# yahoo/CaffeOnSpark

Hardware: AMD Instinct MI355X
Metric: images/sec (higher is better)
Workload: dtype bf16; 1 GPU; model=alexnet(bvlc_reference/CaffeNet), global_batch=256, parallelism=dp1

## Files before the change

### caffeonspark_amd/ops/csrc/elementwise.hip

```cpp

#include "common.h"

namespace cosamd {

typedef unsigned short u16;
typedef unsigned short u16x8 __attribute__((ext_vector_type(8)));
typedef unsigned short u16x4 __attribute__((ext_vector_type(4)));
typedef float f32x4 __attribute__((ext_vector_type(4)));

__device__ __forceinline__ float ldbf(const u16* p) {
  return bf2f(*reinterpret_cast<const bf16*>(p));
}
__device__ __forceinline__ void stbf(u16* p, float v) {
  bf16 b = f2bf(v);
  *p = *reinterpret_cast<u16*>(&b);
}


__global__ void relu_fwd_kernel(const u16* __restrict__ x, u16* __restrict__ y,
                                float slope, int64_t n8, int64_t n) {
  if (blockIdx.x == 0 && threadIdx.x == 0)
    for (int64_t k = n8 * 8; k < n; ++k) {
      float f = ldbf(x + k);
      stbf(y + k, f > 0.f ? f : f * slope);
// ... 121 lines not shown
       i < n; i += (int64_t)gridDim.x * blockDim.x)
    stbf(y + i, ldbf(a + i) * ldbf(b + i));
}


__global__ void sgd_update_kernel(float* __restrict__ p, const float* __restrict__ g,
                                  float* __restrict__ v, float lr, float mu,
                                  float wd, int64_t n4, int64_t n) {
  for (int64_t i = (int64_t)blockIdx.x * blockDim.x + threadIdx.x;
       i < n4; i += (int64_t)gridDim.x * blockDim.x) {
    if (i * 4 + 4 <= n) {
      f32x4 pv = *reinterpret_cast<f32x4*>(p + i * 4);
      f32x4 gv = *reinterpret_cast<const f32x4*>(g + i * 4);
      f32x4 vv = *reinterpret_cast<f32x4*>(v + i * 4);
#pragma unroll
      for (int j = 0; j < 4; ++j) {
        float gg = gv[j] + wd * pv[j];
        vv[j] = mu * vv[j] + lr * gg;
        pv[j] -= vv[j];
      }
      *reinterpret_cast<f32x4*>(v + i * 4) = vv;
      *reinterpret_cast<f32x4*>(p + i * 4) = pv;
    } else {
      for (int64_t k = i * 4; k < n; ++k) {
        float gg = g[k] + wd * p[k];
        v[k] = mu * v[k] + lr * gg;
        p[k] -= v[k];
      }
    }
  }
}


__global__ void bias_act_cast_kernel(const float* __restrict__ in,
                                     const float* __restrict__ bias,
                                     u16* __restrict__ out, int64_t rows,
                                     int cols, int relu) {
  int64_t total = rows * cols;
  for (int64_t i = (int64_t)blockIdx.x * blockDim.x + threadIdx.x;
       i < total; i += (int64_t)gridDim.x * blockDim.x) {
    float v = in[i];
    if (bias != nullptr) v += bias[i % cols];
    if (relu && v < 0.f) v = 0.f;
    stbf(out + i, v);
  }
}

void bias_act_cast(const float* in, const float* bias, void* out,
                   int64_t rows, int cols, bool relu, hipStream_t stream) {
  int64_t total = rows * cols;
  int blocks = (int)hmin<int64_t>(4096, (total + 255) / 256);
  bias_act_cast_kernel<<<blocks, 256, 0, stream>>>(
      in, bias, (u16*)out, rows, cols, relu ? 1 : 0);
}


__global__ void transpose_bf16_kernel(const u16* __restrict__ in,
                                      u16* __restrict__ out,
                                      int R, int C, int tiles_c) {
  __shared__ unsigned lds32[64][67];
  int nblk = gridDim.x;
  int tile = xcd_swizzle(blockIdx.x, nblk);
  int r0 = (tile / tiles_c) * 128;
  int c0 = (tile % tiles_c) * 64;
  int t = threadIdx.x;
  bool interior = (r0 + 128 <= R) && (c0 + 64 <= C);
  int lc8 = (t & 7) * 8;
#pragma unroll
  for (int half = 0; half < 2; ++half) {
    int r2 = (t >> 3) + half * 32;
    int grlo = r0 + 2 * r2, grhi = grlo + 1;
    if (interior) {
      u16x8 vlo = *reinterpret_cast<const u16x8*>(
          in + (int64_t)grlo * C + c0 + lc8);
      u16x8 vhi = *reinterpret_cast<const u16x8*>(
          in + (int64_t)grhi * C + c0 + lc8);
#pragma unroll
      for (int j = 0; j < 8; ++j)
        lds32[r2][lc8 + j] = (unsigned)vlo[j] | ((unsigned)vhi[j] << 16);
    } else {
#pragma unroll
      for (int j = 0; j < 8; ++j) {
        int gc = c0 + lc8 + j;
        u16 lo = (grlo < R && gc < C) ? in[(int64_t)grlo * C + gc] : 0;
        u16 hi = (grhi < R && gc < C) ? in[(int64_t)grhi * C + gc] : 0;
        lds32[r2][lc8 + j] = (unsigned)lo | ((unsigned)hi << 16);
      }
    }
  }
  __syncthreads();
  int cl = t >> 4;
  int lr8 = (t & 15) * 8;
#pragma unroll
  for (int pass = 0; pass < 4; ++pass) {
    int c = cl + pass * 16;
    int gc = c0 + c;
    if (interior) {
      u16x8 v;
#pragma unroll
      for (int m = 0; m < 4; ++m) {
        unsigned pair = lds32[(lr8 >> 1) + m][c];
        v[2 * m] = (u16)(pair & 0xFFFF);
        v[2 * m + 1] = (u16)(pair >> 16);
      }
      *reinterpret_cast<u16x8*>(out + (int64_t)gc * R + r0 + lr8) = v;
    } else if (gc < C) {
// ... 643 lines not shown
```

### caffeonspark_amd/ops/csrc/ext.cpp

```cpp

#include <torch/extension.h>
#include <ATen/hip/HIPContext.h>

#include <cstdint>

typedef struct ihipStream_t* hipStream_t;

namespace cosamd {

void gemm_bf16(const void* A, const void* B, void* C, const float* bias,
               int M, int N, int K, int lda, int ldb, int ldc,
               bool trans_a, bool trans_b, int store_mode, int splitk,
               bool relu, float alpha, int m_alloc, int n_alloc,
               hipStream_t stream);
void gemm_f32(const float* A, const float* B, float* C, const float* bias,
              int M, int N, int K, int64_t lda, int64_t ldb, int64_t ldc,
              bool trans_a, bool trans_b, int splitk, bool relu,
              hipStream_t stream);
void im2col_f32(const float* x, float* col, int N, int H, int W, int P,
                int Q, int R, int S, int sh, int sw, int ph, int pw, int dh,
                int dw, int c0, int Cg, int64_t sN, int64_t sC, int64_t sH,
                int64_t sW, hipStream_t stream);
void col2im_f32(const float* dcol, float* dx, int N, int H, int W, int P,
                int Q, int R, int S, int sh, int sw, int ph, int pw, int dh,
                int dw, int c0, int Cg, int64_t sN, int64_t sC, int64_t sH,
                int64_t sW, hipStream_t stream);
void gemm_conv_fwd(const void* X, const void* B, void* C,
                   const float* bias, const void* zpage, int M, int N,
                   int K, int ldb, int ldc, bool relu, bool accum,
                   const int* geom, int groups, int gs_c, int gs_b,
                   int gs_n, int cfg, int vec, hipStream_t stream);
struct ConvCfg { int id, bm, bn, waves, depth; };
ConvCfg conv_fwd_plan(int M, int N, int K);
int conv_fwd_num_cfgs();
ConvCfg conv_fwd_cfg(int id);
void gemm_conv_dw(const void* A, const void* X, float* C,
                  const void* zpage, int M, int N, int K, int lda, int ldc,
                  int store_mode, int splitk, float alpha, float* db,
                  const int* geom, hipStream_t stream);
void gemm_conv_fwd_sc(const void* X, const void* B, void* C,
                      const float* bias, int M, int N, int K, int ldb,
                      int ldc, bool relu, const int* geom,
                      hipStream_t stream);
void gemm_conv_dw_sc(const void* A, const void* X, float* C, int M,
                     int N, int K, int lda, int ldc, int store_mode,
                     int splitk, float alpha, float* db, const int* geom,
                     hipStream_t stream);
void repack_weights(const int64_t* table, int ndesc, int64_t max_total,
                    hipStream_t stream);
void dw_unpack_acc(const float* dwp, float* arena, int Kout, int Cg,
                   int R, int S, int Kpad, bool accumulate,
                   hipStream_t stream);
void s2d_pack(const void* x, void* out, int N, int H, int W, int C, int st,
              int ph, int pw, int Hp, int Wp, int64_t sN, int64_t sC,
              int64_t sH, int64_t sW, hipStream_t stream);
void s2d_pack_weight(const void* src, void* dst, int Kout, int Cg, int R,
                     int S, int st, int Kpad, hipStream_t stream);
void d2s_pack_weight(const void* src, void* dst, int Ci, int Co, int R,
                     int S, int st, int Kpad, hipStream_t stream);
void d2s_unpack(const void* z, void* y, int N, int Co, int Ho, int Wo,
                int st, int ph, int pw, int Hp, int Wp, int64_t sN,
                int64_t sC, int64_t sH, int64_t sW, hipStream_t stream);
void data_transform(const void* src, int64_t src_bytes, const int64_t* table,
                    const int64_t* table_host, int N, const float* mean,
                    int mean_mode, int64_t mean_numel, int mC, int mH,
                    int mW, float scale, void* out, bool out_bf16, int C,
                    int oh, int ow, int64_t osN, int64_t osC, int64_t osH,
// ... 107 lines not shown
                  int T, int N, int H, int n_alloc_whc, hipStream_t stream);
void lstm_seq_bwd(const void* dy, const void* w_hcT, const void* cont,
                  const void* h, const float* c, const float* act,
                  void* dxg, void* dh_rec, float* dh_f, float* dc_a,
                  float* dc_b, int T, int N, int H, int n_alloc_whcT,
                  hipStream_t stream);
int64_t lstm_step_lds_bytes(int N, int D, int H, int Ds);
void lstm_step(const void* x, const void* h_prev, const void* xs,
               const void* w_xc, const void* w_hc, const void* w_xsc,
               const void* bias, const float* cont, const float* c_prev,
               float* c_out, void* h_out, int N, int D, int H, int Ds,
               hipStream_t stream);
void softmax_loss_fwd(const void* x, const float* label, float* prob,
                      float* rowloss, float* loss, int* count,
                      int64_t nrows, int C, int ignore, bool has_ignore,
                      hipStream_t stream);
void softmax_loss_bwd(const float* prob, const float* label, void* dx,
                      float scale, int64_t nrows, int C, int ignore,
                      bool has_ignore, hipStream_t stream);

}

namespace {

using at::Tensor;

hipStream_t cur_stream() {
  return at::hip::getCurrentHIPStream().stream();
}

#define CHECK_BF16(t) \
  TORCH_CHECK((t).scalar_type() == at::kBFloat16, #t " must be bf16")
#define CHECK_F32(t) \
  TORCH_CHECK((t).scalar_type() == at::kFloat, #t " must be fp32")
#define CHECK_CUDA(t) TORCH_CHECK((t).is_cuda(), #t " must be on GPU")

void py_gemm(Tensor A, Tensor B, Tensor C, c10::optional<Tensor> bias,
             int64_t M, int64_t N, int64_t K, int64_t lda, int64_t ldb,
             int64_t ldc, bool trans_a, bool trans_b, int64_t store_mode,
             int64_t splitk, bool relu, double alpha, int64_t m_alloc,
             int64_t n_alloc) {
  CHECK_CUDA(A); CHECK_BF16(A); CHECK_BF16(B);
  const float* bptr = nullptr;
  if (bias.has_value()) {
    CHECK_F32(bias.value());
    bptr = bias.value().data_ptr<float>();
  }
  cosamd::gemm_bf16(
      A.data_ptr(), B.data_ptr(), C.data_ptr(), bptr, (int)M, (int)N, (int)K, (int)lda, (int)ldb, (int)ldc,
      trans_a, trans_b, (int)store_mode, (int)splitk, relu, (float)alpha,
      (int)m_alloc, (int)n_alloc, cur_stream());
}

int64_t span_f32(const Tensor& t) {
  return (int64_t)(t.storage().nbytes() / sizeof(float)) - t.storage_offset();
}

void py_gemm_f32(Tensor A, Tensor B, Tensor C, c10::optional<Tensor> bias,
                 int64_t M, int64_t N, int64_t K, int64_t lda, int64_t ldb,
                 int64_t ldc, bool trans_a, bool trans_b, int64_t splitk,
                 bool relu) {
  CHECK_CUDA(A); CHECK_CUDA(B); CHECK_CUDA(C);
  CHECK_F32(A); CHECK_F32(B); CHECK_F32(C);
  const int64_t lim = 1ll << 31;
  TORCH_CHECK(M > 0 && N > 0 && K > 0 && M < lim && N < lim && K < lim,
              "gemm_f32: bad M/N/K");
  int64_t ar = trans_a ? K : M, ac = trans_a ? M : K;
  int64_t br = trans_b ? K : N, bc = trans_b ? N : K;
  TORCH_CHECK(lda >= ac && ldb >= bc && ldc >= N,
              "gemm_f32: leading dimension smaller than the row");
  TORCH_CHECK((ar - 1) * lda + ac <= span_f32(A), "gemm_f32: A too small");
  TORCH_CHECK((br - 1) * ldb + bc <= span_f32(B), "gemm_f32: B too small");
  TORCH_CHECK((M - 1) * ldc + N <= span_f32(C), "gemm_f32: C too small");
  TORCH_CHECK(splitk >= 1 && splitk <= 65535, "gemm_f32: bad splitk");
  TORCH_CHECK((N + 127) / 128 <= 65535, "gemm_f32: N too large");
  const float* bptr = nullptr;
  if (bias.has_value()) {
    const Tensor& b = bias.value();
    CHECK_CUDA(b); CHECK_F32(b);
    TORCH_CHECK(b.is_contiguous() && b.numel() >= N,
                "gemm_f32: bias must hold N contiguous floats");
    bptr = b.data_ptr<float>();
  }
  cosamd::gemm_f32(A.data_ptr<float>(), B.data_ptr<float>(),
                   C.data_ptr<float>(), bptr, (int)M, (int)N, (int)K, lda,
                   ldb, ldc, trans_a, trans_b, (int)splitk, relu,
                   cur_stream());
}

void check_conv_f32(const Tensor& x, const Tensor& col, int64_t P, int64_t Q,
                    int64_t R, int64_t S, int64_t sh, int64_t sw, int64_t ph,
                    int64_t pw, int64_t dh, int64_t dw, int64_t c0,
                    int64_t Cg) {
  CHECK_CUDA(x); CHECK_CUDA(col); CHECK_F32(x); CHECK_F32(col);
  TORCH_CHECK(x.dim() == 4, "x must be 4-D");
  const int64_t lim = 1ll << 31;
  int64_t N = x.size(0), C = x.size(1), H = x.size(2), W = x.size(3);
  TORCH_CHECK(N > 0 && H > 0 && W > 0 && N < lim && H < lim && W < lim,
              "bad input shape");
  TORCH_CHECK(P > 0 && Q > 0 && R > 0 && S > 0 && sh > 0 && sw > 0 &&
              ph >= 0 && pw >= 0 && dh > 0 && dw > 0 && c0 >= 0 && Cg > 0 &&
              c0 + Cg <= C, "bad conv geometry");
  TORCH_CHECK(N * P * Q < lim && Cg * R * S < lim, "conv too large");
  int64_t last = 0;
  for (int d = 0; d < 4; ++d) {
    TORCH_CHECK(x.stride(d) >= 0, "negative stride");
// ... 603 lines not shown
                    dw.data_ptr<float>(), idx.numel(), dw.size(1), V,
                    cur_stream());
}

void py_lstm_seq_fwd(Tensor xg, Tensor w_hc, Tensor cont, Tensor h,
                     Tensor c, Tensor act, Tensor h_in, Tensor hg,
                     int64_t T, int64_t N, int64_t H, int64_t n_alloc) {
  CHECK_BF16(xg); CHECK_BF16(w_hc); CHECK_F32(c); CHECK_F32(act);
  CHECK_F32(hg);
  cosamd::lstm_seq_fwd(xg.data_ptr(), w_hc.data_ptr(), cont.data_ptr(),
                       h.data_ptr(), c.data_ptr<float>(),
                       act.data_ptr<float>(), h_in.data_ptr(),
                       hg.data_ptr<float>(), T, N, H, n_alloc,
                       cur_stream());
}

void py_lstm_seq_bwd(Tensor dy, Tensor w_hcT, Tensor cont, Tensor h,
                     Tensor c, Tensor act, Tensor dxg, Tensor dh_rec,
                     Tensor dh_f, Tensor dc_a, Tensor dc_b, int64_t T,
                     int64_t N, int64_t H, int64_t n_alloc) {
  CHECK_BF16(dy); CHECK_BF16(w_hcT); CHECK_F32(dh_f);
  cosamd::lstm_seq_bwd(dy.data_ptr(), w_hcT.data_ptr(), cont.data_ptr(),
                       h.data_ptr(), c.data_ptr<float>(),
                       act.data_ptr<float>(), dxg.data_ptr(),
                       dh_rec.data_ptr(), dh_f.data_ptr<float>(),
                       dc_a.data_ptr<float>(), dc_b.data_ptr<float>(),
                       T, N, H, n_alloc, cur_stream());
}

void py_softmax_loss_fwd(Tensor x, Tensor label, Tensor prob,
                         Tensor rowloss, Tensor loss, Tensor count,
                         int64_t ignore, bool has_ignore) {
  CHECK_BF16(x); CHECK_F32(label); CHECK_F32(prob); CHECK_F32(rowloss);
  TORCH_CHECK(rowloss.is_contiguous() && rowloss.numel() >= x.size(0),
              "rowloss must hold one value per row");
  cosamd::softmax_loss_fwd(x.data_ptr(), label.data_ptr<float>(),
                           prob.data_ptr<float>(),
                           rowloss.data_ptr<float>(), loss.data_ptr<float>(),
                           count.data_ptr<int>(), x.size(0), x.size(1),
                           (int)ignore, has_ignore, cur_stream());
}

void py_softmax_loss_bwd(Tensor prob, Tensor label, Tensor dx, double scale,
                         int64_t ignore, bool has_ignore) {
  cosamd::softmax_loss_bwd(prob.data_ptr<float>(), label.data_ptr<float>(),
                           dx.data_ptr(), scale, prob.size(0), prob.size(1),
                           (int)ignore, has_ignore, cur_stream());
}

}

PYBIND11_MODULE(TORCH_EXTENSION_NAME, m) {
  m.def("gemm", &py_gemm);
  m.def("gemm_f32", &py_gemm_f32);
  m.def("im2col_f32", &py_im2col_f32);
  m.def("col2im_f32", &py_col2im_f32);
  m.def("relu_colsum_bwd", &py_relu_colsum_bwd);
  m.def("relu_db_dense", &py_relu_db_dense);
  m.def("gemm_conv_fwd", &py_gemm_conv_fwd, py::arg("X"), py::arg("B"),
        py::arg("C"), py::arg("bias"), py::arg("zpage"), py::arg("M"),
        py::arg("N"), py::arg("K"), py::arg("ldb"), py::arg("ldc"),
        py::arg("relu"), py::arg("accum"), py::arg("geom"),
        py::arg("groups") = 1, py::arg("gs_c") = 0, py::arg("gs_b") = 0,
        py::arg("gs_n") = 0, py::arg("cfg") = -1, py::arg("vec") = -1);
  m.def("conv_fwd_plan", &py_conv_fwd_plan);
  m.def("conv_fwd_cfgs", &py_conv_fwd_cfgs);
  m.def("gemm_conv_dw", &py_gemm_conv_dw);
  m.def("gemm_conv_fwd_sc", &py_gemm_conv_fwd_sc);
  m.def("gemm_conv_dw_sc", &py_gemm_conv_dw_sc);
  m.def("im2col", &py_im2col);
  m.def("bn_stats", [](Tensor x, Tensor sum, Tensor sq, int64_t rows,
                       int64_t C) {
    cosamd::bn_stats(x.data_ptr(), sum.data_ptr<float>(),
                     sq.data_ptr<float>(), rows, C, cur_stream());
  });
  m.def("bn_bwd_sums", [](Tensor dy, Tensor xhat, Tensor s1, Tensor s2,
                          int64_t rows, int64_t C) {
    cosamd::bn_bwd_sums(dy.data_ptr(), xhat.data_ptr(),
                        s1.data_ptr<float>(), s2.data_ptr<float>(), rows,
                        C, cur_stream());
  });
  m.def("bn_norm", [](Tensor x, Tensor y, Tensor mean, Tensor invstd,
                      int64_t rows, int64_t C) {
    cosamd::bn_norm(x.data_ptr(), y.data_ptr(), mean.data_ptr<float>(),
                    invstd.data_ptr<float>(), rows, C, cur_stream());
  });
  m.def("bn_bwd", [](Tensor xhat, Tensor dy, Tensor dx, Tensor invstd,
                     Tensor s1, Tensor s2, double inv_m, int64_t rows,
                     int64_t C) {
    cosamd::bn_bwd(xhat.data_ptr(), dy.data_ptr(), dx.data_ptr(),
                   invstd.data_ptr<float>(), s1.data_ptr<float>(),
                   s2.data_ptr<float>(), (float)inv_m, rows, C,
                   cur_stream());
  });
  m.def("wino_conv", [](Tensor x, Tensor w, c10::optional<Tensor> bias,
                        Tensor y, Tensor U, Tensor V, Tensor M, int64_t N,
                        int64_t H, int64_t W, int64_t Cin, int64_t K,
                        int64_t wK, int64_t wC, int64_t u_rows_alloc,
                        bool flip, bool relu) {
    cosamd::wino_conv(x.data_ptr(), w.data_ptr<float>(),
                      bias ? bias->data_ptr<float>() : nullptr,
                      y.data_ptr(), U.data_ptr(), V.data_ptr(),
                      M.data_ptr(), N, H, W, Cin, K, wK, wC, u_rows_alloc,
                      flip, relu, cur_stream());
  });
  m.def("im2col_t", [](Tensor x, Tensor colT, int64_t N, int64_t H,
// ... 58 lines not shown
```

### caffeonspark_amd/ops/csrc/gemm.hip

```cpp

#include "common.h"

#include <type_traits>

namespace cosamd {

typedef __bf16 bf16x8 __attribute__((ext_vector_type(8)));
typedef unsigned short short8v __attribute__((ext_vector_type(8)));
typedef float f32x4 __attribute__((ext_vector_type(4)));

constexpr int BM = 128, BN = 128, BK = 32;
constexpr int NTHREADS = 256;

__device__ __forceinline__ int swz_chunk(int row, int chunk) {
  return chunk ^ ((row >> 1) & 3);
}


struct Tile { int bm, bn, tile_m, tile_n; };

template <int TBN, int TBM = BM>
__device__ __forceinline__ Tile decode_tile(int M, int N) {
  int mblocks = (M + TBM - 1) / TBM;
  int nblocks = (N + TBN - 1) / TBN;
// ... 123 lines not shown
        if (relu) {
#pragma unroll
          for (int j = 0; j < 8; ++j) v[j] = v[j] < 0.f ? 0.f : v[j];
        }
        short8v* dst =
            reinterpret_cast<short8v*>(C + (int64_t)grow * ldc + col);
        bf16 o[8];
        if (accum) {
          short8v old = *dst;
          __builtin_memcpy(o, &old, 16);
#pragma unroll
          for (int j = 0; j < 8; ++j) v[j] += bf2f(o[j]);
        }
#pragma unroll
        for (int j = 0; j < 8; ++j) o[j] = f2bf(v[j]);
        short8v out;
        __builtin_memcpy(&out, o, 16);
        *dst = out;
      }
    }
    __builtin_amdgcn_wave_barrier();
  }
}

template <int STORE, bool BIAS, int MF, int MROWS>
__device__ __forceinline__ void epilogue_f32(
    const f32x4 (&acc)[MF][4], float* C, const float* bias, int M, int N,
    int ldc, int tile_m, int tile_n, int wm, int wn, int lane, int relu,
    float alpha) {
  int crow0 = tile_m + wm * MROWS + ((lane >> 4) << 2);
  int ccol0 = tile_n + wn * 64 + (lane & 15);
#pragma unroll
  for (int fm = 0; fm < MF; ++fm) {
#pragma unroll
    for (int fn = 0; fn < 4; ++fn) {
      int col = ccol0 + fn * 16;
      if (col >= N) continue;
      float badd = (BIAS && bias != nullptr) ? bias[col] : 0.f;
#pragma unroll
      for (int r = 0; r < 4; ++r) {
        int row = crow0 + fm * 16 + r;
        if (row >= M) continue;
        float v = acc[fm][fn][r] * alpha;
        if (BIAS) {
          v += badd;
          if (relu && v < 0.f) v = 0.f;
        }
        if (STORE == 1)
          C[(int64_t)row * ldc + col] = v;
        else
          atomicAdd(C + (int64_t)row * ldc + col, v);
      }
    }
  }
}


__device__ __forceinline__ void stage_direct_guarded(
    bf16* lds_, const bf16* g_, int row0, int rows, int ld,
    int k0, int kend, int tid, int nthreads = NTHREADS) {
  auto* lds = reinterpret_cast<unsigned short*>(lds_);
  auto* g = reinterpret_cast<const unsigned short*>(g_);
  for (int slot = tid; slot < 512; slot += nthreads) {
    int row = slot >> 2;
    int kk = (slot & 3) * 8;
    int grow = row0 + row;
    int gk = k0 + kk;
    unsigned short* dst = lds + row * BK + (swz_chunk(row, slot & 3) << 3);
    if (grow < rows && gk + 8 <= kend && ((ld | gk) % 8 == 0)) {
      *reinterpret_cast<short8v*>(dst) =
          *reinterpret_cast<const short8v*>(g + (int64_t)grow * ld + gk);
    } else if (grow < rows) {
#pragma unroll
      for (int j = 0; j < 8; ++j)
        dst[j] = (gk + j < kend) ? g[(int64_t)grow * ld + gk + j] : 0;
    } else {
#pragma unroll
      for (int j = 0; j < 8; ++j) dst[j] = 0;
    }
  }
}


__device__ __forceinline__ void write_kpairs(
    unsigned short* lds, int m0, int kp, const unsigned short (&va)[8],
    const unsigned short (&vb)[8]) {
  int kk = kp * 2;
  int chunk0 = kk >> 3, kin = kk & 7;
#pragma unroll
  for (int j = 0; j < 8; ++j) {
    int row = m0 + j;
    unsigned int packed = (unsigned int)va[j] |
                          ((unsigned int)vb[j] << 16);
    *reinterpret_cast<unsigned int*>(
        lds + row * BK + (swz_chunk(row, chunk0) << 3) + kin) = packed;
  }
}

__device__ __forceinline__ void stage_trans_pair_guarded(
    bf16* lds_, const bf16* g_, int row0, int rows, int ld,
    int k0, int kend, int tid, int nthreads = NTHREADS,
    int tile_rows = BM) {
  auto* lds = reinterpret_cast<unsigned short*>(lds_);
  auto* g = reinterpret_cast<const unsigned short*>(g_);
  int rslots = tile_rows >> 3;
  int nslots = 16 * rslots;
// ... 971 lines not shown
  else
    gemm_conv_fwd_sc_kernel<4><<<grid, dim3(256), 0, stream>>>(
        (const bf16*)X, (const bf16*)B, (bf16*)C, bias, M, N, K, ldb,
        ldc, relu ? 1 : 0, gm);
}

void gemm_conv_dw_sc(const void* A, const void* X, float* C, int M,
                     int N, int K, int lda, int ldc, int store_mode,
                     int splitk, float alpha, float* db, const int* geom,
                     hipStream_t stream) {
  launch_wide_tt((const bf16*)A, C, M, N, K, lda, ldc, store_mode,
                 split_k(K, splitk), alpha, db,
                 BImplicitSC{(const bf16*)X, make_geom(geom)}, stream);
}

void gemm_conv_dw(const void* A, const void* X, float* C,
                  const void* zpage, int M, int N, int K, int lda, int ldc,
                  int store_mode, int splitk, float alpha, float* db,
                  const int* geom, hipStream_t stream) {
  const char* tr_e = getenv("COS_DW_TR");
  bool tr_env = !(tr_e && tr_e[0] == '0');
  CGeom gm = make_geom(geom);
  SplitK sk = split_k(K, splitk);
  bool tr = tr_env && db == nullptr && zpage != nullptr &&
            ((M | lda | gm.C | gm.c0 | gm.Cg | gm.Kcol) % 8 == 0) &&
            (((uintptr_t)A | (uintptr_t)X) % 16 == 0);
  if (!tr) {
    launch_wide_tt((const bf16*)A, C, M, N, K, lda, ldc, store_mode, sk,
                   alpha, db, BImplicit{(const bf16*)X, gm}, stream);
    return;
  }
  int mblocks = (M + BM - 1) / BM, nblocks = (N + WBN - 1) / WBN;
  dim3 grid(mblocks * nblocks, sk.zblocks);
  if (store_mode == 1 && sk.zblocks == 1)
    gemm_conv_dw_tr_kernel<1, DW_TR_DEPTH><<<grid, WNT, 0, stream>>>(
        (const bf16*)A, (const bf16*)X, (const bf16*)zpage, C, M, N, K, lda,
        ldc, sk.ksplit, alpha, gm);
  else
    gemm_conv_dw_tr_kernel<2, DW_TR_DEPTH><<<grid, WNT, 0, stream>>>(
        (const bf16*)A, (const bf16*)X, (const bf16*)zpage, C, M, N, K, lda,
        ldc, sk.ksplit, alpha, gm);
}

void gemm_bf16(const void* A_, const void* B_, void* C, const float* bias,
               int M, int N, int K, int lda, int ldb, int ldc,
               bool trans_a, bool trans_b, int store_mode, int splitk,
               bool relu, float alpha, int m_alloc, int n_alloc,
               hipStream_t stream) {
  gemm_bf16_batched(A_, B_, C, bias, M, N, K, lda, ldb, ldc, trans_a,
                    trans_b, store_mode, splitk, relu, alpha, m_alloc,
                    n_alloc, 1, 0, 0, 0, stream);
}

}
```

### caffeonspark_amd/ops/gpu.py

```python

from __future__ import annotations

import math
import os
import torch

from . import reference

_ext = None


def _pad8(k: int) -> int:
    return (k + 7) // 8 * 8


def _pad32(k: int) -> int:
    return (k + 31) // 32 * 32


def _kpad_dma(k: int) -> int:
    return max(64, _pad32(k))


def _cl(x: torch.Tensor) -> torch.Tensor:
# ... 745 lines not shown
    _check_bf16(x, "deconv input")
    sh, sw = stride
    ph, pw = pad
    dil = dilation[0]
    N, Ci, H, W = x.shape
    G = groups
    Cog, R, S = w.shape[1], w.shape[2], w.shape[3]
    if w.shape[0] != Ci or Ci % G != 0:
        raise ValueError(f"deconv weight {tuple(w.shape)} does not match "
                         f"{Ci} input channels in {G} groups")
    Co = Cog * G
    Ho = sh * (H - 1) + dil * (R - 1) + 1 - 2 * ph
    Wo = sw * (W - 1) + dil * (S - 1) + 1 - 2 * pw
    if Ho <= 0 or Wo <= 0:
        raise ValueError("deconv output is empty")
    d2s = _d2s_geom(N, Ci, Co, H, W, R, S, sh, sw, dil, G)
    if d2s is not None:
        y = _deconv2d_forward_d2s(x, w, b, d2s, Co, R, S, ph, pw, Ho, Wo,
                                  relu)
    else:
        Kcol = R * S * Cog
        shape = (N, Co, Ho, Wo, H, W, R, S, sh, sw, ph, pw, dil, G, Cog,
                 Ci // G, _pad8(Kcol), Kcol)
        y = _deconv2d_forward_col2im(x, w, b, shape, relu)
    if ctx is not None:
        ctx["route"] = "d2s" if d2s is not None else "col2im"
    return y


def deconv2d_backward(x, w, dy, stride, pad, dilation, groups,
                      need_dx=True, need_dw=True, bias=True, ctx=None,
                      dw_out=None, db_out=None):
    _check_bf16(dy, "deconv dy")
    dx = dw = db = None
    c = {}
    if need_dx:
        dx = conv2d_forward(dy, w, None, stride, pad, dilation, groups,
                            ctx=c)
    if need_dw:
        _, dw, _ = conv2d_backward(dy, w, x, stride, pad, dilation, groups,
                                   need_dx=False, need_dw=True, bias=False,
                                   ctx=c, dw_out=dw_out)
    if bias:
        N, Co, Ho, Wo = dy.shape
        dyl = _cl(dy)
        db = db_out if db_out is not None \
            else _scratch_buf((Co,), torch.float32, dy.device)
        _ext.colsum(dyl.permute(0, 2, 3, 1).reshape(N * Ho * Wo, Co), db,
                    N * Ho * Wo, Co, Co)
    return dx, dw, db



def fc_forward(x, w, b, relu=False):
    _check_bf16(x, "fc input")
    x = x.contiguous()
    M, K = x.shape
    Nout = w.shape[0]
    if Nout % 128:
        wb = torch.zeros((_pad128(Nout), K), dtype=torch.bfloat16,
                         device=x.device)
        wb[:Nout] = _as_bf16(w)
        na = wb.shape[0]
        wb = wb[:Nout]
    else:
        wb = _as_bf16(w).contiguous()
        na = Nout
    y = torch.empty((M, Nout), dtype=torch.bfloat16, device=x.device)
    bias_f = b.float().contiguous() if b is not None else None
    mb, nb = (M + 127) // 128, (Nout + 127) // 128
    sk = _splitk_for(mb, nb, K)
    if sk > 1:
        wsp = torch.zeros((M, Nout), dtype=torch.float32, device=x.device)
        _gemm(x, wb, wsp, None, M, Nout, K, K, K, Nout, False, False, 2,
              sk, na=na)
        _ext.bias_act_cast(wsp, bias_f, y, relu)
    else:
        _gemm(x, wb, y, bias_f, M, Nout, K, K, K, Nout, False, False, 0, 1,
              relu=relu, na=na)
    return y


def fc_backward(x, w, dy, need_dx=True, bias=True, dw_out=None,
                db_out=None):
    _check_bf16(dy, "fc dy")
    x = x.contiguous()
    dy = dy.contiguous()
    wb = _as_bf16(w).contiguous()
    M, K = x.shape
    Nout = wb.shape[0]
    dx = dw = db = None
    Np = Nout
    if Nout % 8:
        Np = _pad8(Nout)
        dy_p = _scratch_buf((M, Np), torch.bfloat16, dy.device,
                            zero_each_step=False)
        dy_p[:, :Nout] = dy
        dy = dy_p
        wb_p = _scratch_buf((Np, K), torch.bfloat16, dy.device,
                            zero_each_step=False)
        wb_p[:Nout] = wb
        wb = wb_p
    if need_dx:
        wT = _transpose(wb)
        dx = torch.empty((M, K), dtype=torch.bfloat16, device=x.device)
        mb, nb = (M + 127) // 128, (K + 127) // 128
        sk = _splitk_for(mb, nb, Np)
        if sk > 1:
            wsp = _scratch_buf((M, K), torch.float32, x.device)
            _gemm(dy, wT, wsp, None, M, K, Np, Np, Np, K, False,
                  False, 2, sk, na=_pad128(K))
            _ext.bias_act_cast(wsp, None, dx, False)
        else:
            _gemm(dy, wT, dx, None, M, K, Np, Np, Np, K, False,
                  False, 0, 1, na=_pad128(K))
    sk_tt = _splitk_tt(Nout, K, M)
    arena_dw = dw_out is not None and dw_out.dtype == torch.float32 \
        and dw_out.is_contiguous() and tuple(dw_out.shape) == (Nout, K)
    if sk_tt == 1:
        dwp = dw_out if arena_dw else torch.empty(
            (Nout, K), dtype=torch.float32, device=x.device)
        store_dw = 1
    elif arena_dw:
        dwp = dw_out
        dwp.zero_()
        store_dw = 2
    else:
        dwp = _scratch_buf((Nout, K), torch.float32, x.device)
        store_dw = 2
    fuse_db = bias and K > 128 and \
        bool(int(os.environ.get("COS_FUSE_DB", "0")))
    if fuse_db:
        db = db_out if db_out is not None \
            else _scratch_buf((Nout,), torch.float32, x.device)
    _gemm(dy, x, dwp, db if fuse_db else None, Nout, K, M, Np, K, K,
          True, True, store_dw, sk_tt)
    dw = dwp
    if bias and not fuse_db:
        db = db_out if db_out is not None \
            else _scratch_buf((Nout,), torch.float32, x.device)
        _ext.colsum(dy, db, M, Nout, Np)
    return dx, dw, db



def gemm_f32(A, B, C, bias, M, N, K, lda, ldb, ldc, trans_a=False,
             trans_b=False, splitk=1, relu=False):
    _ext.gemm_f32(A, B, C, bias, M, N, K, lda, ldb, ldc, trans_a, trans_b,
                  splitk, relu)
    return C


def _splitk_f32(M: int, N: int, K: int) -> int:
    tiles = ((M + 127) // 128) * ((N + 127) // 128)
    if tiles >= 256 or K < 1024:
        return 1
# ... 788 lines not shown
```

Measured before the change: 85230 images/sec.

## Add streaming skinny-M FC GEMM kernel with split-K slabs and fused finalize

Adds a dedicated FC GEMM kernel for small batch M (≤256). Each block covers the whole M extent and a 128-wide N tile, and the kernel uses direct global-to-LDS loads, a 4-deep ring buffer and MFMA. Split-K partials go into per-split fp32 slabs that a fused finalize kernel sums while adding bias, applying ReLU and casting to bf16, replacing the atomic split-K plus bias_act_cast path. For dx, the kernel reads W through a transposing LDS read, so the explicit transpose is no longer needed. It adds a slab workspace allocation in the forward pass each call and significant new kernel complexity.

```diff
diff --git a/caffeonspark_amd/ops/csrc/elementwise.hip b/caffeonspark_amd/ops/csrc/elementwise.hip
--- a/caffeonspark_amd/ops/csrc/elementwise.hip
+++ b/caffeonspark_amd/ops/csrc/elementwise.hip
@@ -197,6 +197,58 @@
   int blocks = (int)hmin<int64_t>(4096, (total + 255) / 256);
   bias_act_cast_kernel<<<blocks, 256, 0, stream>>>(
       in, bias, (u16*)out, rows, cols, relu ? 1 : 0);
+}
+
+__global__ void fc_slab_finalize_kernel(const float* __restrict__ slabs,
+                                        int sk, const float* __restrict__ bias,
+                                        u16* __restrict__ out, int M, int N,
+                                        int ldo, int relu, int vec) {
+  int64_t slab = (int64_t)M * N;
+  int64_t start = (int64_t)blockIdx.x * blockDim.x + threadIdx.x;
+  int64_t step = (int64_t)gridDim.x * blockDim.x;
+  if (vec) {
+    int n8 = N / 8;
+    for (int64_t i = start; i < (int64_t)M * n8; i += step) {
+      int row = (int)(i / n8), col = (int)(i - (int64_t)row * n8) * 8;
+      const float* p = slabs + (int64_t)row * N + col;
+      float v[8] = {};
+      for (int s = 0; s < sk; ++s, p += slab) {
+        f32x4 lo = *reinterpret_cast<const f32x4*>(p);
+        f32x4 hi = *reinterpret_cast<const f32x4*>(p + 4);
+#pragma unroll
+        for (int j = 0; j < 4; ++j) { v[j] += lo[j]; v[4 + j] += hi[j]; }
+      }
+      u16x8 o;
+#pragma unroll
+      for (int j = 0; j < 8; ++j) {
+        float f = v[j] + (bias != nullptr ? bias[col + j] : 0.f);
+        if (relu && f < 0.f) f = 0.f;
+        bf16 b = f2bf(f);
+        o[j] = *reinterpret_cast<u16*>(&b);
+      }
+      *reinterpret_cast<u16x8*>(out + (int64_t)row * ldo + col) = o;
+    }
+  } else {
+    for (int64_t i = start; i < slab; i += step) {
+      int row = (int)(i / N), col = (int)(i - (int64_t)row * N);
+      float v = 0.f;
+      for (int s = 0; s < sk; ++s) v += slabs[s * slab + i];
+      if (bias != nullptr) v += bias[col];
+      if (relu && v < 0.f) v = 0.f;
+      stbf(out + (int64_t)row * ldo + col, v);
+    }
+  }
+}
+
+void fc_slab_finalize(const float* slabs, int sk, const float* bias,
+                      void* out, int M, int N, int ldo, bool relu,
+                      hipStream_t stream) {
+  bool vec = N % 8 == 0 && ldo % 8 == 0 &&
+             (((uintptr_t)slabs | (uintptr_t)out) % 16 == 0);
+  int64_t work = vec ? (int64_t)M * (N / 8) : (int64_t)M * N;
+  int blocks = (int)hmin<int64_t>(2048, (work + 255) / 256);
+  fc_slab_finalize_kernel<<<blocks, 256, 0, stream>>>(
+      slabs, sk, bias, (u16*)out, M, N, ldo, relu ? 1 : 0, vec ? 1 : 0);
 }
 
 
diff --git a/caffeonspark_amd/ops/csrc/ext.cpp b/caffeonspark_amd/ops/csrc/ext.cpp
--- a/caffeonspark_amd/ops/csrc/ext.cpp
+++ b/caffeonspark_amd/ops/csrc/ext.cpp
@@ -13,6 +13,15 @@
                bool trans_a, bool trans_b, int store_mode, int splitk,
                bool relu, float alpha, int m_alloc, int n_alloc,
                hipStream_t stream);
+struct FcPlan { int route, bm, bn, depth, sk; };
+FcPlan fc_gemm_plan(int M, int N, int K, int kind, bool aligned);
+int gemm_fc(const void* A, const void* B, void* C, float* slabs,
+            const float* bias, const void* zpage, int M, int N, int K,
+            int lda, int ldb, int ldc, int kind, int sk, bool relu,
+            hipStream_t stream);
+void fc_slab_finalize(const float* slabs, int sk, const float* bias,
+                      void* out, int M, int N, int ldo, bool relu,
+                      hipStream_t stream);
 void gemm_f32(const float* A, const float* B, float* C, const float* bias,
               int M, int N, int K, int64_t lda, int64_t ldb, int64_t ldc,
               bool trans_a, bool trans_b, int splitk, bool relu,
@@ -226,6 +235,78 @@
       (int)m_alloc, (int)n_alloc, cur_stream());
 }
 
+std::vector<int64_t> py_fc_gemm_plan(int64_t M, int64_t N, int64_t K,
+                                     int64_t kind, bool aligned) {
+  cosamd::FcPlan p = cosamd::fc_gemm_plan((int)M, (int)N, (int)K, (int)kind,
+                                          aligned);
+  return {p.route, p.bm, p.bn, p.depth, p.sk};
+}
+
+int64_t py_gemm_fc(Tensor A, Tensor B, Tensor C, c10::optional<Tensor> slabs,
+                   c10::optional<Tensor> bias, Tensor zpage, int64_t M,
+                   int64_t N, int64_t K, int64_t lda, int64_t ldb,
+                   int64_t ldc, int64_t kind, int64_t sk, bool relu) {
+  CHECK_CUDA(A); CHECK_CUDA(B); CHECK_CUDA(C); CHECK_CUDA(zpage);
+  CHECK_BF16(A); CHECK_BF16(B); CHECK_BF16(C); CHECK_BF16(zpage);
+  TORCH_CHECK(zpage.numel() >= 8, "zpage must hold 16 zero bytes");
+  TORCH_CHECK(M > 0 && N > 0 && K > 0 && sk <= 65535, "gemm_fc: bad size");
+  auto span = [](const Tensor& t) {
+    return (int64_t)(t.storage().nbytes() / t.element_size()) -
+           t.storage_offset();
+  };
+  int64_t br = kind == 1 ? K : N, bc = kind == 1 ? N : K;
+  TORCH_CHECK(lda >= K && ldb >= bc && ldc >= N,
+              "gemm_fc: leading dimension smaller than the row");
+  TORCH_CHECK((M - 1) * lda + K <= span(A), "gemm_fc: A too small");
+  TORCH_CHECK((br - 1) * ldb + bc <= span(B), "gemm_fc: B too small");
+  TORCH_CHECK((M - 1) * ldc + N <= span(C), "gemm_fc: C too small");
+  float* sp = nullptr;
+  if (slabs.has_value()) {
+    const Tensor& s = slabs.value();
+    CHECK_CUDA(s); CHECK_F32(s);
+    int64_t want = sk > 0 ? sk : cosamd::fc_gemm_plan(
+        (int)M, (int)N, (int)K, (int)kind, true).sk;
+    int64_t ksplit = ((K + want - 1) / want + 31) / 32 * 32;
+    int64_t need = (K + ksplit - 1) / ksplit;
+    TORCH_CHECK(s.is_contiguous() && s.numel() >= need * M * N,
+                "gemm_fc: slabs must hold one [M, N] slab per split");
+    sp = s.data_ptr<float>();
+  }
+  const float* bptr = nullptr;
+  if (bias.has_value()) {
+    const Tensor& b = bias.value();
+    CHECK_CUDA(b); CHECK_F32(b);
+    TORCH_CHECK(b.is_contiguous() && b.numel() >= N,
+                "gemm_fc: bias must hold N contiguous floats");
+    bptr = b.data_ptr<float>();
+  }
+  return cosamd::gemm_fc(A.data_ptr(), B.data_ptr(), C.data_ptr(), sp, bptr,
+                         zpage.data_ptr(), (int)M, (int)N, (int)K, (int)lda,
+                         (int)ldb, (int)ldc, (int)kind, (int)sk, relu,
+                         cur_stream());
+}
+
+void py_fc_slab_finalize(Tensor slabs, int64_t sk, c10::optional<Tensor> bias,
+                         Tensor out, int64_t M, int64_t N, int64_t ldo,
+                         bool relu) {
+  CHECK_CUDA(slabs); CHECK_F32(slabs); CHECK_CUDA(out); CHECK_BF16(out);
+  TORCH_CHECK(sk >= 1 && slabs.is_contiguous() &&
+              slabs.numel() >= sk * M * N, "fc_slab_finalize: slabs too small");
+  TORCH_CHECK(ldo >= N && (M - 1) * ldo + N <=
+              (int64_t)(out.storage().nbytes() / 2) - out.storage_offset(),
+              "fc_slab_finalize: out too small");
+  const float* bptr = nullptr;
+  if (bias.has_value()) {
+    CHECK_F32(bias.value());
+    TORCH_CHECK(bias.value().is_contiguous() && bias.value().numel() >= N,
+                "fc_slab_finalize: bias must hold N contiguous floats");
+    bptr = bias.value().data_ptr<float>();
+  }
+  cosamd::fc_slab_finalize(slabs.data_ptr<float>(), (int)sk, bptr,
+                           out.data_ptr(), (int)M, (int)N, (int)ldo, relu,
+                           cur_stream());
+}
+
 int64_t span_f32(const Tensor& t) {
   return (int64_t)(t.storage().nbytes() / sizeof(float)) - t.storage_offset();
 }
@@ -935,6 +1016,10 @@
 
 PYBIND11_MODULE(TORCH_EXTENSION_NAME, m) {
   m.def("gemm", &py_gemm);
+  m.def("fc_gemm_plan", &py_fc_gemm_plan, py::arg("M"), py::arg("N"),
+        py::arg("K"), py::arg("kind"), py::arg("aligned") = true);
+  m.def("gemm_fc", &py_gemm_fc);
+  m.def("fc_slab_finalize", &py_fc_slab_finalize);
   m.def("gemm_f32", &py_gemm_f32);
   m.def("im2col_f32", &py_im2col_f32);
   m.def("col2im_f32", &py_col2im_f32);
diff --git a/caffeonspark_amd/ops/csrc/gemm.hip b/caffeonspark_amd/ops/csrc/gemm.hip
--- a/caffeonspark_amd/ops/csrc/gemm.hip
+++ b/caffeonspark_amd/ops/csrc/gemm.hip
@@ -199,6 +199,40 @@
           atomicAdd(C + (int64_t)row * ldc + col, v);
       }
     }
+  }
+}
+
+template <int NCOLS>
+constexpr int f32_slab_floats() { return 16 * (NCOLS + 4); }
+
+template <int MF, int NF, int NCOLS>
+__device__ __forceinline__ void epilogue_f32_vec(
+    const f32x4 (&acc)[MF][NF], float* slab, float* C, int M, int N, int ldc,
+    int row0, int col0, int lane, float alpha) {
+  constexpr int LD = NCOLS + 4;
+  constexpr int GPR = NCOLS / 4;
+  constexpr int TASKS = 16 * GPR;
+  static_assert(TASKS % 64 == 0, "whole wave-instructions per band");
+  int wr = (lane >> 4) << 2, wc = lane & 15;
+#pragma unroll
+  for (int fm = 0; fm < MF; ++fm) {
+#pragma unroll
+    for (int fn = 0; fn < NF; ++fn)
+#pragma unroll
+      for (int r = 0; r < 4; ++r)
+        slab[(wr + r) * LD + fn * 16 + wc] = acc[fm][fn][r] * alpha;
+    __builtin_amdgcn_wave_barrier();
+#pragma unroll
+    for (int t0 = 0; t0 < TASKS; t0 += 64) {
+      int t = t0 + lane;
+      int row = t / GPR, cg = t - row * GPR;
+      int grow = row0 + fm * 16 + row;
+      int col = col0 + cg * 4;
+      if (grow < M && col < N)
+        *reinterpret_cast<f32x4*>(C + (int64_t)grow * ldc + col) =
+            *reinterpret_cast<const f32x4*>(slab + row * LD + cg * 4);
+    }
+    __builtin_amdgcn_wave_barrier();
   }
 }
 
@@ -1276,4 +1310,254 @@
                     n_alloc, 1, 0, 0, 0, stream);
 }
 
-}
+
+constexpr int FC_BN = 128;
+constexpr int FC_DEPTH = 4;
+
+struct FcPlan { int route, bm, bn, depth, sk; };
+
+__device__ __forceinline__ bf16x8 ds_read_b128_asm(unsigned addr) {
+  bf16x8 v;
+  asm volatile("ds_read_b128 %0, %1" : "=v"(v) : "v"(addr) : "memory");
+  return v;
+}
+
+template <int TBM, bool TRB, int DEPTH>
+__global__ __launch_bounds__(512, 1) void gemm_fc_kernel(
+    const bf16* __restrict__ A, const bf16* __restrict__ B,
+    const bf16* __restrict__ zpage, bf16* __restrict__ Cb,
+    float* __restrict__ Cs, const float* __restrict__ bias, int M, int N,
+    int K, int lda, int ldb, int ldc, int ksplit, int relu, int vec) {
+  constexpr int WM = TBM / 64, WN = 8 / WM;
+  using Cfg = TileCfg<TBM, FC_BN, WM, WN>;
+  constexpr int MF = Cfg::MF, NF = Cfg::NF, NCOLS = Cfg::NCOLS;
+  constexpr int A_BYTES = TBM * BK * 2, B_BYTES = FC_BN * BK * 2;
+  constexpr int STAGE = A_BYTES + B_BYTES;
+  constexpr int A_CPW = Cfg::A_CPW;
+  static_assert(MF == 4 && Cfg::B_CHUNKS == 8, "one B chunk per wave");
+  static_assert(DEPTH * STAGE >= vec_slab_floats<Cfg>() * 4 &&
+                DEPTH * STAGE >= 8 * f32_slab_floats<NCOLS>() * 4,
+                "the epilogue slabs fit in the ring");
+  __shared__ __attribute__((aligned(16))) unsigned char smem[DEPTH * STAGE];
+
+  int tile_n = blockIdx.x * FC_BN;
+  int k_begin = blockIdx.y * ksplit;
+  int k_end = min(K, k_begin + ksplit);
+
+  int tid = threadIdx.x;
+  int wave = tid >> 6, lane = tid & 63;
+  int wm = wave / WN, wn = wave % WN;
+
+  const unsigned short* as = reinterpret_cast<const unsigned short*>(A);
+  const unsigned short* bs = reinterpret_cast<const unsigned short*>(B);
+  int64_t a_off[A_CPW];
+  int a_kk[A_CPW];
+  bool a_ok[A_CPW];
+#pragma unroll
+  for (int it = 0; it < A_CPW; ++it) {
+    int row = (wave * A_CPW + it) * 16 + (lane >> 2);
+    a_kk[it] = swz_chunk(row, lane & 3) << 3;
+    a_ok[it] = row < M;
+    a_off[it] = (int64_t)row * lda + a_kk[it];
+  }
+  int64_t b_off;
+  int b_kk;
+  bool b_ok;
+  if (TRB) {
+    int srow = wave * 4 + (lane >> 4);
+    int sch = (dw_tr_off(srow, lane & 15) >> 4) & 15;
+    int col = tile_n + sch * 8;
+    b_kk = srow;
+    b_ok = col < N;
+    b_off = (int64_t)srow * ldb + col;
+  } else {
+    int row = wave * 16 + (lane >> 2);
+    b_kk = swz_chunk(row, lane & 3) << 3;
+    b_ok = tile_n + row < N;
+    b_off = (int64_t)(tile_n + row) * ldb + b_kk;
+  }
+  typedef const __attribute__((address_space(1))) unsigned int* gptr;
+  typedef __attribute__((address_space(3))) unsigned int* lptr;
+  auto keep_v = [](int64_t v) {
+    asm volatile("" : "+v"(v));
+    return v;
+  };
+  auto stage = [&](int slot, int k0) {
+    unsigned char* base = smem + slot * STAGE;
+#pragma unroll
+    for (int it = 0; it < A_CPW; ++it) {
+      bool ok = a_ok[it] & (k0 + a_kk[it] < k_end);
+      int64_t off = keep_v(a_off[it] + k0);
+      const void* src = ok ? (const void*)(as + off) : (const void*)zpage;
+      __builtin_amdgcn_global_load_lds(
+          (gptr)src, (lptr)(base + (wave * A_CPW + it) * 1024), 16, 0, 0);
+    }
+    bool ok = b_ok & (k0 + b_kk < k_end);
+    int64_t off = keep_v(b_off + (TRB ? (int64_t)k0 * ldb : (int64_t)k0));
+    const void* src = ok ? (const void*)(bs + off) : (const void*)zpage;
+    __builtin_amdgcn_global_load_lds(
+        (gptr)src, (lptr)(base + A_BYTES + wave * 1024), 16, 0, 0);
+  };
+
+  int lrow = lane & 15, lchunk = lane >> 4;
+  int a_addr[MF], b_addr[NF][2];
+#pragma unroll
+  for (int f = 0; f < MF; ++f) {
+    int ra = wm * 64 + f * 16 + lrow;
+    a_addr[f] = ra * 64 + (swz_chunk(ra, lchunk) << 4);
+  }
+  if (TRB) {
+    int fq = (lane >> 2) & 3, fp = lane & 3;
+#pragma unroll
+    for (int f = 0; f < NF; ++f)
+#pragma unroll
+      for (int h = 0; h < 2; ++h)
+        b_addr[f][h] = A_BYTES +
+            dw_tr_off(8 * lchunk + 4 * h + fq,
+                      (wn * NCOLS + f * 16) / 8 + (fp >> 1)) + 8 * (fp & 1);
+  } else {
+#pragma unroll
+    for (int f = 0; f < NF; ++f) {
+      int rb = wn * NCOLS + f * 16 + lrow;
+      b_addr[f][0] = b_addr[f][1] =
+          A_BYTES + rb * 64 + (swz_chunk(rb, lchunk) << 4);
+    }
+  }
+  unsigned lds0 = (unsigned)(uintptr_t)(
+      (__attribute__((address_space(3))) unsigned char*)smem);
+
+  f32x4 acc[MF][NF] = {};
+
+  constexpr int PF = DEPTH - 1;
+  constexpr int VMCNT = (A_CPW + 1) * (PF - 1);
+  int tiles = (k_end - k_begin + BK - 1) / BK;
+#pragma unroll
+  for (int p = 0; p < PF; ++p) stage(p, k_begin + p * BK);
+  int cur = 0;
+  for (int i = 0; i < tiles; ++i) {
+    wait_vmcnt<VMCNT>();
+    __builtin_amdgcn_sched_barrier(0);
+    __builtin_amdgcn_s_barrier();
+    int nxt = cur == 0 ? DEPTH - 1 : cur - 1;
+    stage(nxt, k_begin + (i + PF) * BK);
+    unsigned img = lds0 + cur * STAGE;
+    bf16x8 afrag[MF], bfrag[NF];
+    if (TRB) {
+      bf16x4 br[NF][2];
+#pragma unroll
+      for (int f = 0; f < NF; ++f)
+#pragma unroll
+        for (int h = 0; h < 2; ++h)
+          br[f][h] = ds_read_tr16(img + b_addr[f][h]);
+#pragma unroll
+      for (int f = 0; f < MF; ++f) afrag[f] = ds_read_b128_asm(img + a_addr[f]);
+      asm volatile("s_waitcnt lgkmcnt(0)" ::: "memory");
+#pragma unroll
+      for (int f = 0; f < NF; ++f) {
+        asm volatile("" : "+v"(br[f][0]), "+v"(br[f][1]));
+        bfrag[f] = __builtin_shufflevector(br[f][0], br[f][1], 0, 1, 2, 3, 4,
+                                           5, 6, 7);
+      }
+    } else {
+#pragma unroll
+      for (int f = 0; f < NF; ++f)
+        bfrag[f] = ds_read_b128_asm(img + b_addr[f][0]);
+#pragma unroll
+      for (int f = 0; f < MF; ++f) afrag[f] = ds_read_b128_asm(img + a_addr[f]);
+      asm volatile("s_waitcnt lgkmcnt(0)" ::: "memory");
+#pragma unroll
+      for (int f = 0; f < NF; ++f) asm volatile("" : "+v"(bfrag[f]));
+    }
+#pragma unroll
+    for (int f = 0; f < MF; ++f) asm volatile("" : "+v"(afrag[f]));
+    __builtin_amdgcn_s_setprio(1);
+#pragma unroll
+    for (int fm = 0; fm < MF; ++fm)
+#pragma unroll
+      for (int fn = 0; fn < NF; ++fn)
+        acc[fm][fn] = __builtin_amdgcn_mfma_f32_16x16x32_bf16(
+            afrag[fm], bfrag[fn], acc[fm][fn], 0, 0, 0);
+    __builtin_amdgcn_s_setprio(0);
+    cur = cur + 1 == DEPTH ? 0 : cur + 1;
+  }
+  wait_vmcnt<0>();
+
+  float* lds_f = reinterpret_cast<float*>(smem);
+  if (Cs != nullptr) {
+    float* slab = Cs + (int64_t)blockIdx.y * M * N;
+    if (vec) {
+      __syncthreads();
+      epilogue_f32_vec<MF, NF, NCOLS>(
+          acc, lds_f + wave * f32_slab_floats<NCOLS>(), slab, M, N, N,
+          wm * 64, tile_n + wn * NCOLS, lane, 1.f);
+    } else {
+      int crow0 = wm * 64 + (lchunk << 2), ccol0 = tile_n + wn * NCOLS + lrow;
+#pragma unroll
+      for (int fm = 0; fm < MF; ++fm)
+#pragma unroll
+        for (int fn = 0; fn < NF; ++fn)
+#pragma unroll
+          for (int r = 0; r < 4; ++r) {
+            int row = crow0 + fm * 16 + r, col = ccol0 + fn * 16;
+            if (row < M && col < N)
+              slab[(int64_t)row * N + col] = acc[fm][fn][r];
+          }
+    }
+  } else if (vec) {
+    __syncthreads();
+    epilogue_bf16_vec<Cfg>(acc, lds_f, Cb, bias, M, N, ldc, 0, tile_n, wm, wn,
+                           wave, lane, relu, 0);
+  } else {
+    epilogue_bf16<MF, 64, NF, NCOLS>(acc, Cb, bias, M, N, ldc, 0, tile_n, wm,
+                                     wn, lane, relu, 1.f, std::false_type{});
+  }
+}
+
+FcPlan fc_gemm_plan(int M, int N, int K, int kind, bool aligned) {
+  const char* e = getenv("COS_FC_STREAM");
+  bool on = !(e && e[0] == '0');
+  FcPlan p{0, 0, FC_BN, FC_DEPTH, 1};
+  if (!on || !aligned || M < 1 || M > 256 || N < 1 || K < 8 || K % 8 != 0 ||
+      (kind == 1 && N % 8 != 0) || (kind != 0 && kind != 1))
+    return p;
+  p.route = 1;
+  p.bm = M <= 128 ? 128 : 256;
+  int ntiles = (N + FC_BN - 1) / FC_BN;
+  p.sk = hmax(1, hmin(hmin(K / 256, 256 / ntiles), 16));
+  return p;
+}
+
+int gemm_fc(const void* A, const void* B, void* C, float* slabs,
+            const float* bias, const void* zpage, int M, int N, int K,
+            int lda, int ldb, int ldc, int kind, int sk, bool relu,
+            hipStream_t stream) {
+  bool aligned = (((uintptr_t)A | (uintptr_t)B | (uintptr_t)zpage) % 16 ==
+                  0) && ((lda | ldb) % 8 == 0);
+  FcPlan p = fc_gemm_plan(M, N, K, kind, aligned);
+  if (!p.route || zpage == nullptr || lda < K || ldc < N ||
+      ldb < (kind == 1 ? N : K))
+    throw std::runtime_error("gemm_fc: shape or alignment outside the "
+                             "streaming kernel (see fc_gemm_plan)");
+  SplitK s = split_k(K, sk > 0 ? sk : p.sk);
+  if (s.zblocks > 1 && slabs == nullptr)
+    throw std::runtime_error("gemm_fc: split-K needs the slab workspace");
+  float* cs = s.zblocks > 1 ? slabs : nullptr;
+  int vec = cs != nullptr
+                ? (N % 4 == 0 && (uintptr_t)cs % 16 == 0)
+                : ((N | ldc) % 8 == 0 && (uintptr_t)C % 16 == 0 &&
+                   (bias == nullptr || (uintptr_t)bias % 16 == 0));
+  dim3 grid((N + FC_BN - 1) / FC_BN, s.zblocks);
+#define COS_FC_CASE(TBM, TRB)                                               \
+  gemm_fc_kernel<TBM, TRB, FC_DEPTH><<<grid, 512, 0, stream>>>(             \
+      (const bf16*)A, (const bf16*)B, (const bf16*)zpage, (bf16*)C, cs,     \
+      bias, M, N, K, lda, ldb, ldc, s.ksplit, relu ? 1 : 0, vec)
+  if (p.bm == 128) {
+    if (kind == 1) COS_FC_CASE(128, true); else COS_FC_CASE(128, false);
+  } else {
+    if (kind == 1) COS_FC_CASE(256, true); else COS_FC_CASE(256, false);
+  }
+#undef COS_FC_CASE
+  return s.zblocks;
+}
+
+}
diff --git a/caffeonspark_amd/ops/gpu.py b/caffeonspark_amd/ops/gpu.py
--- a/caffeonspark_amd/ops/gpu.py
+++ b/caffeonspark_amd/ops/gpu.py
@@ -821,19 +821,54 @@
 
 
 
+def _fc_aligned(*ts):
+    return all(t.dim() == 2 and (t.stride(1) == 1 or t.shape[1] == 1)
+               and t.data_ptr() % 16 == 0 and t.stride(0) % 8 == 0
+               and t.stride(0) >= t.shape[1] for t in ts)
+
+
+def fc_gemm_plan(M, N, K, kind, aligned=True):
+    r, bm, bn, depth, sk = _ext.fc_gemm_plan(
+        M, N, K, {"fwd": 0, "dx": 1}[kind], aligned)
+    return ("stream" if r else "legacy"), bm, bn, depth, sk
+
+
+def _fc_stream(a, wb, out, bias_f, kind, relu, sk, slabs=None):
+    M, K = a.shape
+    N = out.shape[1]
+    if sk > 1 and slabs is None:
+        slabs = torch.empty((sk, M, N), dtype=torch.float32,
+                            device=a.device)
+    wrote = _ext.gemm_fc(a, wb, out, slabs if sk > 1 else None, bias_f,
+                         _zpage(a.device), M, N, K, a.stride(0),
+                         wb.stride(0), out.stride(0),
+                         {"fwd": 0, "dx": 1}[kind], sk, relu)
+    if wrote > 1:
+        _ext.fc_slab_finalize(slabs, wrote, bias_f, out, M, N,
+                              out.stride(0), relu)
+    return out
+
+
 def fc_forward(x, w, b, relu=False):
     _check_bf16(x, "fc input")
     x = x.contiguous()
     M, K = x.shape
     Nout = w.shape[0]
+    w16 = _as_bf16(w)
+    route, _, _, _, sk = fc_gemm_plan(M, Nout, K, "fwd",
+                                      _fc_aligned(x, w16))
+    if route == "stream":
+        y = torch.empty((M, Nout), dtype=torch.bfloat16, device=x.device)
+        bias_f = b.float().contiguous() if b is not None else None
+        return _fc_stream(x, w16, y, bias_f, "fwd", relu, sk)
     if Nout % 128:
         wb = torch.zeros((_pad128(Nout), K), dtype=torch.bfloat16,
                          device=x.device)
-        wb[:Nout] = _as_bf16(w)
+        wb[:Nout] = w16
         na = wb.shape[0]
         wb = wb[:Nout]
     else:
-        wb = _as_bf16(w).contiguous()
+        wb = w16.contiguous()
         na = Nout
     y = torch.empty((M, Nout), dtype=torch.bfloat16, device=x.device)
     bias_f = b.float().contiguous() if b is not None else None
@@ -855,7 +890,8 @@
     _check_bf16(dy, "fc dy")
     x = x.contiguous()
     dy = dy.contiguous()
-    wb = _as_bf16(w).contiguous()
+    w16 = _as_bf16(w)
+    wb = w16.contiguous()
     M, K = x.shape
     Nout = wb.shape[0]
     dx = dw = db = None
@@ -870,7 +906,16 @@
                             zero_each_step=False)
         wb_p[:Nout] = wb
         wb = wb_p
+    dx_route, dx_sk = "legacy", 1
     if need_dx:
+        dx_route, _, _, _, dx_sk = fc_gemm_plan(
+            M, K, Np, "dx", _fc_aligned(dy, wb, w16))
+    if need_dx and dx_route == "stream":
+        dx = torch.empty((M, K), dtype=torch.bfloat16, device=x.device)
+        slabs = _scratch_buf((dx_sk, M, K), torch.float32, x.device,
+                             zero_each_step=False) if dx_sk > 1 else None
+        _fc_stream(dy, wb, dx, None, "dx", False, dx_sk, slabs)
+    elif need_dx:
         wT = _transpose(wb)
         dx = torch.empty((M, K), dtype=torch.bfloat16, device=x.device)
         mb, nb = (M + 127) // 128, (K + 127) // 128
```

Result: faster. 90020 images/sec (median of 6 runs) (+5.6%).
